# ultralytics/yolov5

Measured on NVIDIA H100. Metric: images/sec @640 (forward + NMS), higher is better.
Workload: dtype bf16

## Files before the change

include/y5b200.h:

```cpp
#ifndef Y5B200_H
#define Y5B200_H
#include <stdint.h>

#if defined(__GNUC__)
#define Y5_API __attribute__((visibility("default")))
#else
#define Y5_API
#endif

#ifdef __cplusplus
extern "C" {
#endif

#define Y5_F16 0
#define Y5_BF16 1
#define Y5_F32 2
#define Y5_U8 3

#define Y5_E_INVALID (-1)
#define Y5_E_UNSUPPORTED (-2)
#define Y5_E_DRIVER (-3)

#define Y5_ACT_NONE 0
#define Y5_ACT_SILU 1
// ... 3 lines not shown
int64_t y5_launch_count(void);

typedef struct y5_conv_desc {
    const void* in;
    int32_t in_pitch;
    int32_t batch, in_h, in_w, in_c;
    const void* weight;
    const float* bias;
    void* out;
    int32_t out_pitch;
    int32_t out_c;
    const void* residual;
    int32_t res_pitch;
    int32_t ksize, stride, pad;
    int32_t act;
    int32_t dtype;
    int32_t block_k;
    int32_t block_n;
    int32_t kw;
    int32_t pad_w;
    int64_t in_x_stride;
    int64_t in_y_stride;
    int64_t in_n_stride;
    int32_t a_mode;
    int32_t reserved;
} y5_conv_desc;

int y5_conv_pick(int32_t in_c, int32_t out_c, int64_t m_rows, int32_t* block_k, int32_t* block_n);

typedef struct y5_conv_plan y5_conv_plan;
int y5_conv_plan_create(const y5_conv_desc* desc, y5_conv_plan** plan);
int y5_conv_plan_run(const y5_conv_plan* plan, void* stream);
void y5_conv_plan_destroy(y5_conv_plan* plan);
int y5_conv_bn_silu_fwd(const y5_conv_desc* desc, void* stream);
int y5_conv_direct_fwd(const y5_conv_desc* desc, void* stream);

typedef struct y5_detect_desc {
    const void* in;
    int32_t in_pitch;
    int32_t batch, ny, nx, in_c;
    const void* weight;
    const float* bias;
    void* raw;
    void* z;
    int32_t z_rows, z_row0;
    int32_t na, no, nc;
    float stride;
    float anchor_wh[8];
    int32_t dtype;
    int32_t block_k;
} y5_detect_desc;
typedef struct y5_detect_plan y5_detect_plan;
int y5_detect_plan_create(const y5_detect_desc* desc, y5_detect_plan** plan);
int y5_detect_plan_run(const y5_detect_plan* plan, void* stream);
int y5_detect_plan_run_to(const y5_detect_plan* plan, void* raw, void* z, void* stream);
void y5_detect_plan_destroy(y5_detect_plan* plan);

int y5_stem_s2d(const void* img, int32_t img_dtype, void* out, int32_t out_dtype, int32_t batch, int32_t h, int32_t w,
                int32_t out_row_px, int32_t out_x_off, void* stream);
int y5_sppf_pool(const void* x, int32_t x_pitch, void* y1, void* y2, void* y3, int32_t y_pitch, int32_t batch, int32_t h,
                 int32_t w, int32_t c, int32_t ksize, int32_t dtype, void* stream);
int y5_upsample2x(const void* x, int32_t x_pitch, void* y, int32_t y_pitch, int32_t batch, int32_t h, int32_t w, int32_t c,
                  int32_t dtype, void* stream);
int y5_copy_view(const void* x, int32_t x_pitch, void* y, int32_t y_pitch, int64_t pixels, int32_t c, int32_t dtype,
                 void* stream);
int y5_nhwc_to_nchw(const void* x, int32_t x_pitch, void* y, int32_t batch, int32_t h, int32_t w, int32_t c, int32_t dtype,
// ... 277 lines not shown
```

yolov5_b200/_lib.py:

```python
from __future__ import annotations

import ctypes as C
import os

import torch

_HERE = os.path.dirname(os.path.abspath(__file__))
LIB_PATH = os.environ.get("Y5B200_LIB") or os.path.join(_HERE, "liby5b200.so")

Y5_F16, Y5_BF16, Y5_F32, Y5_U8 = 0, 1, 2, 3
ACT_NONE, ACT_SILU = 0, 1

_DTYPE = {torch.float16: Y5_F16, torch.bfloat16: Y5_BF16, torch.float32: Y5_F32, torch.uint8: Y5_U8}


def dtype_code(dt: torch.dtype) -> int:
    try:
        return _DTYPE[dt]
    except KeyError:
        raise TypeError(f"y5b200: unsupported dtype {dt}") from None


class ConvDesc(C.Structure):
    _fields_ = [
# ... 109 lines not shown
    ]


class AugLabel(C.Structure):
    _fields_ = [
        ("cls", C.c_float), ("x", C.c_float), ("y", C.c_float), ("w", C.c_float), ("h", C.c_float),
        ("tile_w", C.c_float), ("tile_h", C.c_float), ("pad_w", C.c_float), ("pad_h", C.c_float),
        ("image", C.c_int32), ("mosaic", C.c_int32), ("flags", C.c_int32),
    ]


AUG_CLIP, AUG_IN_XYXY, AUG_OUT_XYXY = 1, 2, 4


class AugSegment(C.Structure):
    _fields_ = [("point_offset", C.c_int32), ("n_points", C.c_int32)]


SEG_POINTS, SEG_I32 = 1000, 4

OPT_INV_SCALE, OPT_MAX_NORM, OPT_EMA_DECAY, OPT_EMA_TAU, OPT_EMA_UPDATES, OPT_OUT_NORM, OPT_OUT_SKIPPED, OPT_GROUPS = 0, 1, 2, 3, 4, 5, 6, 8
ADAM_LR, ADAM_BETA1, ADAM_BETA2, ADAM_EPS, ADAM_WEIGHT_DECAY, ADAM_DECOUPLED, ADAM_STRIDE = 0, 1, 2, 3, 4, 5, 8

_P = C.c_void_p
_I32, _I64, _F = C.c_int32, C.c_int64, C.c_float
SIGNATURES = {
    "y5_version": (_I32, []),
    "y5_last_error": (C.c_char_p, []),
    "y5_launch_count": (_I64, []),
    "y5_conv_pick": (_I32, [_I32, _I32, _I64, C.POINTER(_I32), C.POINTER(_I32)]),
    "y5_conv_plan_create": (_I32, [C.POINTER(ConvDesc), C.POINTER(_P)]),
    "y5_conv_plan_run": (_I32, [_P, _P]),
    "y5_conv_plan_destroy": (None, [_P]),
    "y5_conv_bn_silu_fwd": (_I32, [C.POINTER(ConvDesc), _P]),
    "y5_conv_direct_fwd": (_I32, [C.POINTER(ConvDesc), _P]),
    "y5_detect_plan_create": (_I32, [C.POINTER(DetectDesc), C.POINTER(_P)]),
    "y5_detect_plan_run": (_I32, [_P, _P]),
    "y5_detect_plan_run_to": (_I32, [_P, _P, _P, _P]),
    "y5_detect_plan_destroy": (None, [_P]),
    "y5_stem_s2d": (_I32, [_P, _I32, _P, _I32, _I32, _I32, _I32, _I32, _I32, _P]),
    "y5_sppf_pool": (_I32, [_P, _I32, _P, _P, _P, _I32, _I32, _I32, _I32, _I32, _I32, _I32, _P]),
    "y5_upsample2x": (_I32, [_P, _I32, _P, _I32, _I32, _I32, _I32, _I32, _I32, _P]),
    "y5_copy_view": (_I32, [_P, _I32, _P, _I32, _I64, _I32, _I32, _P]),
    "y5_nhwc_to_nchw": (_I32, [_P, _I32, _P, _I32, _I32, _I32, _I32, _I32, _P]),
    "y5_nms_workspace_bytes": (_I64, [C.POINTER(NmsParams)]),
    "y5_nms_batched": (_I32, [C.POINTER(NmsParams), _P, _P, _P, _P, _P, _I64, _P]),
    "y5_box_iou": (_I32, [_P, _I32, _P, _I32, _F, _P, _P]),
    "y5_loss_workspace_bytes": (_I64, [C.POINTER(LossParams)]),
    "y5_loss_fwd_bwd": (_I32, [C.POINTER(LossParams), C.POINTER(_P), _P, _P, _P, C.POINTER(_P), _P, _I64, _P]),
    "y5_loss_read_targets": (_I32, [C.POINTER(LossParams), _P, _I32, _P, _P, _P, _P]),
    "y5_seg_loss_workspace_bytes": (_I64, [C.POINTER(LossParams)]),
    "y5_seg_loss_fwd_bwd_scaled": (_I32, [C.POINTER(LossParams), C.POINTER(_P), _P, _P, _P, _I32, _I64, _I64, _I64, _I64, _I32, _I32, _I32,
                                          _P, _I32, _I32, _I32, _I32, _P, C.POINTER(_P), _P, _P, _P, _I64, _P]),
    "y5_seg_loss_read_targets": (_I32, [C.POINTER(LossParams), _P, _I32, _P, _P, _P, _P]),
    "y5_conv_wgrad": (_I32, [C.POINTER(WgradDesc), _P]),
    "y5_bn_workspace_bytes": (_I64, [_I32]),
    "y5_bn_stats": (_I32, [_P, _I32, _I64, _I32, _I32, _P, _P]),
    "y5_bn_act_fwd": (_I32, [_P, _I32, _P, _I32, _I64, _I32, _I32, _P, _P, _P, _P, _I32, _P, _F, _F, _P, _P, _P, _I32, _P]),
    "y5_upsample2x_bwd": (_I32, [_P, _I32, _P, _I32, _I32, _I32, _I32, _I32, _I32, _P]),
    "y5_sppf_bwd_workspace_bytes": (_I64, [_I32, _I32, _I32, _I32]),
    "y5_sppf_pool_bwd": (_I32, [_P, _I32, _P, _I32, _P, _I32, _I32, _I32, _I32, _I32, _I32, _I32, _P, _P]),
    "y5_bn_act_bwd": (_I32, [_P, _I32, _P, _I32, _P, _I32, _I64, _I32, _I32, _P, _P, _P, _P, _I32, _P, _P, _P, _P]),
    "y5_col_sum": (_I32, [_P, _I32, _I64, _I32, _I32, _P, _P, _P]),
    "y5_weight_pack": (_I32, [_P, _I32, _I32, _I32, _I32, _P, _I32, _P, _I32, _I32, _P]),
    "y5_weight_pack_chunk_elems": (_I32, []),
    "y5_weight_pack_multi": (_I32, [_P, _P, _P, _I32, _I32, _P]),
# ... 75 lines not shown
```

yolov5_b200/csrc/conv_gemm.cu:

```cuda
#include <cstdio>
#include <cstdlib>
#include <cstring>
#include <mutex>

#include "../../include/y5b200.h"
#include "common.cuh"
#include "host_util.h"
#include "wgmma.cuh"

namespace y5 {

constexpr int kBlockM = 128;
constexpr int kConsumers = 2;
constexpr int kConsumerThreads = 128 * kConsumers;
constexpr int kThreads = 128 + kConsumerThreads;
constexpr int kMaxStages = 8;
constexpr int kHeadN = 128;

enum AMode { A_LINEAR = 0, A_IM2COL = 1, A_PATCH = 2 };

struct ConvParams {
    int M, N;
    int num_m_tiles;
    int num_m_super, num_n_tiles;
    int kh, kw, c_chunks;
    int block_k;
    int a_mode;
    int Ho, Wo, HoWo, stride, pad_h, pad_w;
    int tw, th, tiles_x, tiles_y;
    int b_grouped;
    int patch_pw;
    int cluster_n;
    uint32_t stg_bytes;
    uint32_t b_sub_bytes;
    float rcp_per_img, rcp_tiles_x, rcp_HoWo, rcp_Wo;
    int a_stages, b_stages;
    uint32_t a_sub_bytes, a_stage_bytes, b_stage_bytes;
    int is_bf16, act;
    const float* bias;
    int bias_n;
    void* out;
    int out_pitch;
    const void* res;
    int res_pitch;
    void* raw;
    void* z;
    int na, no, nc, nx, z_rows, z_row0;
    float det_stride;
    float anchor_wh[8];
};

struct SmemLayout {
    uint32_t off_a, off_b, off_out, off_bias, off_bars, total;
};

__host__ __device__ inline SmemLayout smem_layout(int epi, int no, int bias_n, int a_stages, int b_stages, uint32_t a_bytes,
                                                   uint32_t b_bytes, uint32_t stg_bytes) {
    SmemLayout L;
    uint32_t o = 0;
    L.off_a = o;
    o += a_stages * a_bytes;
    L.off_b = o;
    o += b_stages * b_bytes;
    o = (o + 1023) & ~1023u;
    L.off_out = o;
    if (epi == 1) o += 4 * ((kBlockM * no * 2 + 1023) & ~1023u);
    else o += stg_bytes;
    L.off_bias = o;
    o += ((bias_n + 3) & ~3) * 4;
    o = (o + 7) & ~7u;
    L.off_bars = o;
    o += 4 * kMaxStages * 8;
    L.total = o;
    return L;
}

__device__ __forceinline__ int fdiv(int n, int d, float rd) {
    if (n >= (1 << 23)) return n / d;
    int q = __float2int_rz(__int2float_rz(n) * rd);
    const int r = n - q * d;
    if (r >= d) ++q;
    else if (r < 0) --q;
    return q;
}

template <int BLOCK_N, int MT, int KS, bool BF16>
__device__ __forceinline__ void mma_batch(float (&acc)[MT][BLOCK_N / 2], uint32_t a_lo, uint32_t a_sub16, uint32_t a_hi, uint32_t b_lo,
                                          uint32_t b_hi, uint32_t scale_first) {
    wgmma_fence();
#pragma unroll
    for (int k = 0; k < KS; ++k)
#pragma unroll
        for (int mi = 0; mi < MT; ++mi)
            Wgmma<BLOCK_N>::template run<BF16, 0, 0>(acc[mi], gmma_desc(a_lo + mi * a_sub16 + 2 * k, a_hi), gmma_desc(b_lo + 2 * k, b_hi),
                                                     k == 0 ? scale_first : 1u);
    wgmma_commit();
}

template <int BLOCK_N, int EPI, int MT, bool OPT, bool BF16>
__global__ void __launch_bounds__(kThreads, 1)
conv_gemm_kernel(const __grid_constant__ CUtensorMap tmA, const __grid_constant__ CUtensorMap tmB, const ConvParams p) {
    static_assert(MT * BLOCK_N <= 256, "accumulators: at most 128 fp32 registers per consumer thread");
    constexpr int kAcc = BLOCK_N / 2;

    extern __shared__ __align__(1024) uint8_t smem_raw[];
    uint8_t* smem = reinterpret_cast<uint8_t*>((reinterpret_cast<uintptr_t>(smem_raw) + 1023) & ~uintptr_t(1023));
    const SmemLayout L = smem_layout(EPI, p.no, p.bias_n, p.a_stages, p.b_stages, p.a_stage_bytes, p.b_stage_bytes, p.stg_bytes);
    uint8_t* sA = smem + L.off_a;
    uint8_t* sB = smem + L.off_b;
    float* sBias = reinterpret_cast<float*>(smem + L.off_bias);
    uint64_t* a_full = reinterpret_cast<uint64_t*>(smem + L.off_bars);
    uint64_t* a_empty = a_full + kMaxStages;
    uint64_t* b_full = a_empty + kMaxStages;
    uint64_t* b_empty = b_full + kMaxStages;

    const int warp = threadIdx.x >> 5;
    const int lane = threadIdx.x & 31;
    const int csize = OPT ? static_cast<int>(cluster_nctarank()) : 1;
    const uint32_t crank = OPT ? cluster_ctarank() : 0u;

    if (threadIdx.x == 0) {
        tma_prefetch_desc(&tmA);
        tma_prefetch_desc(&tmB);
        for (int s = 0; s < kMaxStages; ++s) {
            mbar_init(&a_full[s], 1);
            mbar_init(&a_empty[s], kConsumers);
            mbar_init(&b_full[s], 1);
            mbar_init(&b_empty[s], kConsumers * csize);
        }
        fence_barrier_init();
    }
    if (threadIdx.x >= 128)
        for (int i = threadIdx.x - 128; i < p.bias_n; i += kConsumerThreads) {
            const float b = i < p.N ? __ldg(p.bias + i) : 0.0f;
            sBias[i] = (EPI == 0 && p.act) ? 0.5f * b : b;
        }
    __syncthreads();
    if (csize > 1) cluster_sync_all();
    griddep_wait();
    griddep_launch_dependents();

    const int nn = p.num_n_tiles;
    const int num_tiles = ((p.num_m_super + csize - 1) / csize) * nn;
    const int tile0 = blockIdx.x / csize, tile_step = gridDim.x / csize;
    const uint32_t row_bytes = p.block_k * 2;
    const bool patch = p.a_mode == A_PATCH;
    const bool wide = OPT && p.patch_pw > 0;
    const int grp = wide ? p.kh * p.kw : (patch ? p.kh : 1);
    const int num_groups = wide ? p.c_chunks : (patch ? p.c_chunks * p.kw : p.kh * p.kw * p.c_chunks);

    if (warp < 4) {
        setmaxnreg_dec<56>();
    }
    if (warp == 0) {
        int as = 0, bs = 0;
        uint32_t aph = 0, bph = 0;
        for (int tile = tile0; tile < num_tiles; tile += tile_step) {
            const int ms = (tile / nn) * csize + static_cast<int>(crank);
            const int n0 = (tile - (tile / nn) * nn) * BLOCK_N;
            int img[MT], y0[MT], x0[MT];
#pragma unroll
            for (int mi = 0; mi < MT; ++mi) {
                const int mt = ms * MT + mi;
                img[mi] = y0[mi] = x0[mi] = 0;
                if (p.a_mode == A_IM2COL) {
                    const int m0 = mt * kBlockM;
                    img[mi] = fdiv(m0, p.HoWo, p.rcp_HoWo);
                    const int rem = m0 - img[mi] * p.HoWo;
                    const int oy = fdiv(rem, p.Wo, p.rcp_Wo);
                    y0[mi] = oy * p.stride - p.pad_h;
                    x0[mi] = (rem - oy * p.Wo) * p.stride - p.pad_w;
                } else if (patch) {
                    const int per_img = p.tiles_x * p.tiles_y;
                    img[mi] = fdiv(mt, per_img, p.rcp_per_img);
                    const int rem = mt - img[mi] * per_img;
                    const int ty = fdiv(rem, p.tiles_x, p.rcp_tiles_x);
                    y0[mi] = ty * p.th - p.pad_h;
                    x0[mi] = (rem - ty * p.tiles_x) * p.tw - p.pad_w;
                }
            }
            auto issue_group = [&](int cc, int s, int r0) {
                mbar_wait(&a_empty[as], aph ^ 1);
                if (elect_one()) {
                    mbar_arrive_expect_tx(&a_full[as], p.a_stage_bytes);
#pragma unroll
                    for (int mi = 0; mi < MT; ++mi) {
                        uint8_t* a_dst = sA + as * p.a_stage_bytes + mi * p.a_sub_bytes;
                        if (wide) {
                            if (mi == 0) tma_load_4d(&tmA, &a_full[as], a_dst, cc * p.block_k, x0[0], y0[0], img[0]);
                        } else if (p.a_mode == A_LINEAR) tma_load_2d(&tmA, &a_full[as], a_dst, cc * p.block_k, (ms * MT + mi) * kBlockM);
                        else if (p.a_mode == A_IM2COL)
                            tma_load_im2col_4d(&tmA, &a_full[as], a_dst, cc * p.block_k, x0[mi], y0[mi], img[mi], static_cast<uint16_t>(s),
                                               static_cast<uint16_t>(r0));
                        else tma_load_4d(&tmA, &a_full[as], a_dst, cc * p.block_k, x0[mi] + s, y0[mi], img[mi]);
                    }
                }
                __syncwarp();
                if (++as == p.a_stages) { as = 0; aph ^= 1; }
                for (int j = 0; j < grp; ++j) {
                    const int r = patch ? j : r0;
                    const int kb = wide ? j * p.c_chunks + cc : (r * p.kw + s) * p.c_chunks + cc;
                    const bool stage_first = !p.b_grouped || j == 0, stage_last = !p.b_grouped || j == grp - 1;
                    if (stage_first) mbar_wait(&b_empty[bs], bph ^ 1);
                    if (elect_one()) {
                        if (stage_first) mbar_arrive_expect_tx(&b_full[bs], p.b_stage_bytes);
                        uint8_t* b_dst = sB + bs * p.b_stage_bytes + (p.b_grouped ? j * p.b_sub_bytes : 0u);
                        if (csize == 1) tma_load_2d(&tmB, &b_full[bs], b_dst, kb * p.block_k, n0);
                        else {
                            const int slice_rows = BLOCK_N / csize;
                            tma_load_2d_mcast(&tmB, &b_full[bs], b_dst + crank * slice_rows * row_bytes, kb * p.block_k,
                                              n0 + static_cast<int>(crank) * slice_rows, static_cast<uint16_t>((1u << csize) - 1u));
                        }
                    }
                    __syncwarp();
                    if (stage_last && ++bs == p.b_stages) { bs = 0; bph ^= 1; }
                }
            };
            if (wide) {
                for (int cc = 0; cc < p.c_chunks; ++cc) issue_group(cc, 0, 0);
            } else if (patch) {
                for (int cc = 0; cc < p.c_chunks; ++cc)
                    for (int s = 0; s < p.kw; ++s) issue_group(cc, s, 0);
            } else {
                for (int r = 0; r < p.kh; ++r)
                    for (int s = 0; s < p.kw; ++s)
                        for (int cc = 0; cc < p.c_chunks; ++cc) issue_group(cc, s, r);
            }
        }
    } else if (warp >= 4) {
    setmaxnreg_inc<224>();
    const int wg = (warp >> 2) - 1;
    const int ct = threadIdx.x - 128;
    const int wrow = wg * 64 + (warp & 3) * 16 + (lane >> 2);
    const int ccol = 2 * (lane & 3);
    const bool signal = (threadIdx.x & 127) == 0;
    constexpr bool bf16 = BF16;
    const uint32_t dhi = gmma_desc_hi(row_bytes);
    const uint32_t a_hi = wide ? (dhi & ~0x3FFFu) | (((static_cast<uint32_t>(p.patch_pw) * row_bytes) >> 4) & 0x3FFFu) : dhi;
    const uint32_t a_base = gmma_desc_lo(smem_u32(sA) + (wide ? wg * 8 * p.patch_pw : wg * 64) * row_bytes), b_base = gmma_desc_lo(smem_u32(sB));
    const uint32_t row16 = row_bytes >> 4;
    const uint32_t a_stage16 = p.a_stage_bytes >> 4, b_stage16 = p.b_stage_bytes >> 4, a_sub16 = p.a_sub_bytes >> 4;
    const uint32_t b_sub16 = p.b_sub_bytes >> 4;
    const uint32_t a_shift16 = patch ? (p.tw * row_bytes) >> 4 : 0;
    const int k_steps = p.block_k / 16;
    const int per_img = p.tiles_x * p.tiles_y;
    const int tw_shift = patch ? __ffs(p.tw) - 1 : 0;
    int as = 0, bs = 0, head_set = 0;
    uint32_t aph = 0, bph = 0;
    float acc[MT][kAcc];
#pragma unroll
    for (int mi = 0; mi < MT; ++mi)
#pragma unroll
        for (int i = 0; i < kAcc; ++i) acc[mi][i] = 0.0f;

    int pend_as = 0, pend_bs = 0;
    bool pend_a_last = false, pend_b_last = false;
    auto release_pending = [&]() {
        if (!signal) return;
        if (pend_b_last) {
            if (csize == 1) mbar_arrive(&b_empty[pend_bs]);
            else
                for (int r = 0; r < csize; ++r) mbar_arrive_cluster(mapa_u32(&b_empty[pend_bs], static_cast<uint32_t>(r)));
        }
        if (pend_a_last) mbar_arrive(&a_empty[pend_as]);
    };

    for (int tile = tile0; tile < num_tiles; tile += tile_step) {
        const int ms = (tile / nn) * csize + static_cast<int>(crank);
        const int nt = tile - (tile / nn) * nn;
        const int n0 = nt * BLOCK_N;
        for (int g = 0; g < num_groups; ++g) {
            mbar_wait(&a_full[as], aph);
            const uint32_t a_stage_lo = a_base + as * a_stage16;
            uint32_t a_lo = a_stage_lo;
            for (int j = 0; j < grp; ++j) {
                if (wide) {
                    const int tr = j / p.kw, ts = j - tr * p.kw;
                    a_lo = a_stage_lo + (tr * p.patch_pw + ts) * row16;
                }
                const bool stage_first = !p.b_grouped || j == 0, stage_last = !p.b_grouped || j == grp - 1;
                if (stage_first) mbar_wait(&b_full[bs], bph);
                const uint32_t b_lo = b_base + bs * b_stage16 + (p.b_grouped ? j * b_sub16 : 0u);
                const uint32_t scale_first = (g | j) != 0 ? 1u : 0u;
#pragma unroll
                for (int mi = 0; mi < MT; ++mi) fence_regs(acc[mi]);
                switch (k_steps) {
                    case 4: mma_batch<BLOCK_N, MT, 4, BF16>(acc, a_lo, a_sub16, a_hi, b_lo, dhi, scale_first); break;
                    case 2: mma_batch<BLOCK_N, MT, 2, BF16>(acc, a_lo, a_sub16, a_hi, b_lo, dhi, scale_first); break;
                    default: mma_batch<BLOCK_N, MT, 1, BF16>(acc, a_lo, a_sub16, a_hi, b_lo, dhi, scale_first); break;
                }
                wgmma_wait<1>();
#pragma unroll
                for (int mi = 0; mi < MT; ++mi) fence_regs(acc[mi]);
                if (g | j) release_pending();
                pend_as = as;
                pend_a_last = j == grp - 1;
                pend_bs = bs;
                pend_b_last = stage_last;
                if (stage_last && ++bs == p.b_stages) { bs = 0; bph ^= 1; }
                a_lo += a_shift16;
            }
            if (++as == p.a_stages) { as = 0; aph ^= 1; }
        }
        wgmma_wait<0>();
#pragma unroll
        for (int mi = 0; mi < MT; ++mi) fence_regs(acc[mi]);
        release_pending();

        if (EPI == 0) {
            const bool staged = OPT && p.stg_bytes != 0;
            const uint32_t stg_pitch = BLOCK_N * 2 + 16;
            uint8_t* stg = smem + L.off_out + wg * 64 * stg_pitch;
            auto pixel_of = [&](int mt, int row) -> long long {
                if (patch) {
                    const int img = fdiv(mt, per_img, p.rcp_per_img);
                    const int rem = mt - img * per_img;
                    const int tyi = fdiv(rem, p.tiles_x, p.rcp_tiles_x);
                    const int oy = tyi * p.th + (row >> tw_shift), ox = (rem - tyi * p.tiles_x) * p.tw + (row & ((1 << tw_shift) - 1));
                    return (mt < p.num_m_tiles && oy < p.Ho && ox < p.Wo) ? static_cast<long long>(img) * p.HoWo + oy * p.Wo + ox : -1;
                }
                const long long m = static_cast<long long>(mt) * kBlockM + row;
                return m < p.M ? m : -1;
            };
            constexpr int kRows = 2 * MT, kWords = (OPT ? 128 : 256) / BLOCK_N;
            constexpr int kBatch = kWords < 1 ? 1 : (kWords < kRows ? kWords : kRows);
            const bool has_res = p.res != nullptr;
#pragma unroll
            for (int q0 = 0; q0 < kRows; q0 += kBatch) {
                uint32_t rv[kBatch][BLOCK_N / 8];
                long long gp[kBatch];
#pragma unroll
                for (int q = 0; q < kBatch; ++q) gp[q] = pixel_of(ms * MT + (q0 + q) / 2, wrow + 8 * ((q0 + q) & 1));
                if (has_res) {
#pragma unroll
                    for (int q = 0; q < kBatch; ++q) {
                        const uint16_t* rp = reinterpret_cast<const uint16_t*>(p.res) + (gp[q] < 0 ? 0 : gp[q] * p.res_pitch) + n0 + ccol;
#pragma unroll
                        for (int j = 0; j < BLOCK_N / 8; ++j)
                            rv[q][j] = (gp[q] >= 0 && n0 + 8 * j < p.N) ? *reinterpret_cast<const uint32_t*>(rp + 8 * j) : 0u;
                    }
// ... 166 lines not shown

int pick_block_n(int out_c, int64_t m_rows) {
    int bn, mt;
    pick_tile(out_c, m_rows > 0 ? (m_rows + kBlockM - 1) / kBlockM : 1, &bn, &mt);
    return bn;
}

template <int BN, int EPI, int MT, bool OPT>
cudaError_t launch_conv(const CUtensorMap& a, const CUtensorMap& b, const ConvParams& p, int grid, int cluster, uint32_t smem,
                        cudaStream_t st) {
    auto* kernel = p.is_bf16 ? conv_gemm_kernel<BN, EPI, MT, OPT, true> : conv_gemm_kernel<BN, EPI, MT, OPT, false>;
    const cudaError_t attr_err = ensure_dyn_smem(reinterpret_cast<const void*>(kernel), 227 * 1024);
    if (attr_err != cudaSuccess) return attr_err;
    count_launch();
    if (cluster == 1) return launch_pdl(kernel, dim3(grid), dim3(kThreads), smem, st, a, b, p);
    static const bool pdl = [] { const char* e = getenv("Y5_PDL"); return !(e && e[0] == '0'); }();
    cudaLaunchConfig_t cfg{};
    cfg.gridDim = dim3(grid);
    cfg.blockDim = dim3(kThreads);
    cfg.dynamicSmemBytes = smem;
    cfg.stream = st;
    cudaLaunchAttribute attr[2];
    attr[0].id = cudaLaunchAttributeClusterDimension;
    attr[0].val.clusterDim.x = cluster;
    attr[0].val.clusterDim.y = 1;
    attr[0].val.clusterDim.z = 1;
    attr[1].id = cudaLaunchAttributeProgrammaticStreamSerialization;
    attr[1].val.programmaticStreamSerializationAllowed = 1;
    cfg.attrs = attr;
    cfg.numAttrs = pdl ? 2 : 1;
    return cudaLaunchKernelEx(&cfg, kernel, a, b, p);
}

struct PlanCommon {
    CUtensorMap tmA, tmB;
    ConvParams p;
    int block_n, epi, mt, grid, cluster;
    uint32_t smem_bytes;
};

int finish_plan(PlanCommon& pc, int block_n, int epi, int mt, int cluster = 1) {
    ConvParams& p = pc.p;
    p.cluster_n = cluster;
    p.a_stage_bytes = mt * p.a_sub_bytes;
    if (p.patch_pw > 0) p.a_stage_bytes = static_cast<uint32_t>(p.th + p.kh - 1) * p.patch_pw * p.block_k * 2;
    p.num_m_super = (p.num_m_tiles + mt - 1) / mt;
    p.num_n_tiles = epi == 1 ? p.na : (p.N + block_n - 1) / block_n;
    p.bias_n = p.num_n_tiles * block_n;
    const uint32_t budget = 225 * 1024 - 1024;
    const bool patch = p.a_mode == A_PATCH;
    int a_st = 0, b_st = 0;
    if (!patch) {
        for (int s = kMaxStages; s >= 2; --s)
            if (smem_layout(epi, p.no, p.bias_n, s, s, p.a_stage_bytes, p.b_stage_bytes, p.stg_bytes).total <= budget) { a_st = b_st = s; break; }
    } else {
        const int b_min = p.b_grouped ? 2 : 3, b_max = p.b_grouped ? 4 : kMaxStages;
        for (int a = 3; a >= 2 && !a_st; --a)
            for (int b = b_max; b >= b_min; --b)
                if (smem_layout(epi, p.no, p.bias_n, a, b, p.a_stage_bytes, p.b_stage_bytes, p.stg_bytes).total <= budget) { a_st = a; b_st = b; break; }
    }
    if (a_st < 2 || b_st < 2) return set_error(Y5_E_UNSUPPORTED, "conv tile does not fit shared memory (block_n %d a %u b %u)", block_n,
                                                p.a_stage_bytes, p.b_stage_bytes);
    p.a_stages = a_st;
    p.b_stages = b_st;
    pc.smem_bytes = smem_layout(epi, p.no, p.bias_n, a_st, b_st, p.a_stage_bytes, p.b_stage_bytes, p.stg_bytes).total + 1024;
    pc.block_n = block_n;
    pc.epi = epi;
    pc.mt = mt;
    pc.cluster = cluster;
    const long long tiles = static_cast<long long>((p.num_m_super + cluster - 1) / cluster) * p.num_n_tiles;
    const int max_clusters = sm_count() / cluster;
    pc.grid = static_cast<int>(tiles < max_clusters ? tiles : max_clusters) * cluster;
    return 0;
}

int run_plan(const PlanCommon& pc, cudaStream_t st) {
    cudaError_t e = cudaErrorInvalidValue;
    const bool opt = pc.cluster > 1 || pc.p.patch_pw > 0 || pc.p.stg_bytes > 0;
    const int key = (opt ? 100000 : 0) + pc.epi * 10000 + pc.block_n * 10 + pc.mt;
    switch (key) {
        case 324: e = launch_conv<32, 0, 4, false>(pc.tmA, pc.tmB, pc.p, pc.grid, pc.cluster, pc.smem_bytes, st); break;
        case 642: e = launch_conv<64, 0, 2, false>(pc.tmA, pc.tmB, pc.p, pc.grid, pc.cluster, pc.smem_bytes, st); break;
        case 1281: e = launch_conv<128, 0, 1, false>(pc.tmA, pc.tmB, pc.p, pc.grid, pc.cluster, pc.smem_bytes, st); break;
        case 1282: e = launch_conv<128, 0, 2, false>(pc.tmA, pc.tmB, pc.p, pc.grid, pc.cluster, pc.smem_bytes, st); break;
        case 2561: e = launch_conv<256, 0, 1, false>(pc.tmA, pc.tmB, pc.p, pc.grid, pc.cluster, pc.smem_bytes, st); break;
        case 11281: e = launch_conv<kHeadN, 1, 1, false>(pc.tmA, pc.tmB, pc.p, pc.grid, pc.cluster, pc.smem_bytes, st); break;
        case 100324: e = launch_conv<32, 0, 4, true>(pc.tmA, pc.tmB, pc.p, pc.grid, pc.cluster, pc.smem_bytes, st); break;
        case 100642: e = launch_conv<64, 0, 2, true>(pc.tmA, pc.tmB, pc.p, pc.grid, pc.cluster, pc.smem_bytes, st); break;
        case 101281: e = launch_conv<128, 0, 1, true>(pc.tmA, pc.tmB, pc.p, pc.grid, pc.cluster, pc.smem_bytes, st); break;
        case 101282: e = launch_conv<128, 0, 2, true>(pc.tmA, pc.tmB, pc.p, pc.grid, pc.cluster, pc.smem_bytes, st); break;
        case 102561: e = launch_conv<256, 0, 1, true>(pc.tmA, pc.tmB, pc.p, pc.grid, pc.cluster, pc.smem_bytes, st); break;
        default: return set_error(Y5_E_UNSUPPORTED, "conv: no kernel for block_n %d mt %d epi %d", pc.block_n, pc.mt, pc.epi);
    }
    if (e != cudaSuccess) return set_error(int(e), "conv_gemm launch failed: %s", cudaGetErrorString(e));
    return 0;
}

bool aligned16(const void* p) { return (reinterpret_cast<uintptr_t>(p) & 15) == 0; }

struct Geo {
    int kh, kw, pad_h, pad_w, Ho, Wo;
    long long xs, ys, ns;
};
Geo geometry(const y5_conv_desc* d) {
    Geo g;
    g.kh = d->ksize;
    g.kw = d->kw ? d->kw : d->ksize;
    g.pad_h = d->pad;
    g.pad_w = d->kw ? d->pad_w : d->pad;
    g.xs = d->in_x_stride ? d->in_x_stride : d->in_pitch;
    g.ys = d->in_y_stride ? d->in_y_stride : static_cast<long long>(d->in_w) * g.xs;
    g.ns = d->in_n_stride ? d->in_n_stride : static_cast<long long>(d->in_h) * g.ys;
    g.Ho = (d->in_h + 2 * g.pad_h - g.kh) / d->stride + 1;
    g.Wo = (d->in_w + 2 * g.pad_w - g.kw) / d->stride + 1;
    return g;
}

}

struct y5_conv_plan {
    PlanCommon pc;
};
struct y5_detect_plan {
    PlanCommon pc;
};

extern "C" Y5_API int y5_conv_pick(int32_t in_c, int32_t out_c, int64_t m_rows, int32_t* block_k, int32_t* block_n) {
    if (in_c <= 0 || out_c <= 0) return set_error(Y5_E_INVALID, "y5_conv_pick: non-positive channel count");
    if (block_k) *block_k = pick_block_k(in_c);
    if (block_n) *block_n = pick_block_n(out_c, m_rows);
    return 0;
// ... 106 lines not shown
            const double eff8 = (double)g.Wo * g.Ho / ((double)tx8 * 8 * ty16 * 16);
            if ((d->reserved & 128) && !(d->reserved & 32) && row_bytes == 128 && g.kw > 1 && (mt_sel == 1 || (mt_sel == 2 && tx8 % 2 == 0)) &&
                eff8 >= best_eff - 1e-9) {
                p.tw = 8;
                p.th = 16;
                p.patch_pw = 8 * mt_sel + 8;
            }
        }
        if (!p.patch_pw && g.kh > 1 && bn <= 128) {
            p.b_grouped = 1;
            p.b_stage_bytes = g.kh * p.b_sub_bytes;
        }
        p.tiles_x = (g.Wo + p.tw - 1) / p.tw;
        p.tiles_y = (g.Ho + p.th - 1) / p.th;
        p.rcp_tiles_x = 1.0f / static_cast<float>(p.tiles_x);
        p.rcp_per_img = 1.0f / static_cast<float>(p.tiles_x * p.tiles_y);
        p.num_m_tiles = d->batch * p.tiles_x * p.tiles_y;
        p.a_sub_bytes = p.patch_pw ? 8 * row_bytes : (p.th + g.kh - 1) * p.tw * row_bytes;
        cuuint64_t dims[4] = {(cuuint64_t)d->in_c, (cuuint64_t)d->in_w, (cuuint64_t)d->in_h, (cuuint64_t)d->batch};
        cuuint64_t str[3] = {(cuuint64_t)g.xs * 2, (cuuint64_t)g.ys * 2, (cuuint64_t)g.ns * 2};
        cuuint32_t box[4] = {(cuuint32_t)bk, (cuuint32_t)(p.patch_pw ? p.patch_pw : p.tw), (cuuint32_t)(p.th + g.kh - 1), 1};
        e = encode_tiled(&pc.tmA, d->dtype, d->in, 4, dims, str, box, sw, "A patch");
    }
    if (e) { delete plan; return e; }
    const uint64_t ktot = static_cast<uint64_t>(p.kh) * p.kw * p.c_chunks * bk;
    {
        cuuint64_t dims[2] = {ktot, (cuuint64_t)d->out_c};
        cuuint64_t str[1] = {ktot * 2};
        cuuint32_t box[2] = {(cuuint32_t)bk, (cuuint32_t)(bn / cl_sel)};
        e = encode_tiled(&pc.tmB, d->dtype, d->weight, 2, dims, str, box, sw, "B");
    }
    if (e) { delete plan; return e; }
    p.stg_bytes = ((d->reserved & 8) && !(d->reserved & 16)) ? static_cast<uint32_t>(kConsumers * 64 * (bn * 2 + 16)) : 0u;
    int e2 = finish_plan(pc, bn, 0, mt_sel, cl_sel);
    if (e2 && p.stg_bytes) {
        p.stg_bytes = 0;
        e2 = finish_plan(pc, bn, 0, mt_sel, cl_sel);
    }
    if (e2) { delete plan; return e2; }
    *out = plan;
    return 0;
}

extern "C" Y5_API int y5_conv_plan_run(const y5_conv_plan* plan, void* stream) {
    if (!plan) return set_error(Y5_E_INVALID, "conv: null plan");
    return run_plan(plan->pc, static_cast<cudaStream_t>(stream));
}
extern "C" Y5_API void y5_conv_plan_destroy(y5_conv_plan* plan) { delete plan; }

extern "C" Y5_API int y5_conv_bn_silu_fwd(const y5_conv_desc* d, void* stream) {
    y5_conv_plan* plan = nullptr;
    if (int e = y5_conv_plan_create(d, &plan)) return e;
    const int e = y5_conv_plan_run(plan, stream);
    y5_conv_plan_destroy(plan);
    return e;
}

extern "C" Y5_API int y5_conv_direct_fwd(const y5_conv_desc* d, void* stream) {
    if (int e = validate_conv(d)) return e;
    const Geo g = geometry(d);
    const int bk = d->block_k ? d->block_k : pick_block_k(d->in_c);
    const int cin_pad = (d->in_c + bk - 1) / bk * bk;
    const long long total = static_cast<long long>(d->batch) * g.Ho * g.Wo * d->out_c;
    const int threads = 256;
    const long long blocks = (total + threads - 1) / threads;
    conv_direct_kernel<<<static_cast<unsigned>(blocks), threads, 0, static_cast<cudaStream_t>(stream)>>>(
        static_cast<const uint16_t*>(d->in), g.xs, g.ys, g.ns, d->batch, d->in_h, d->in_w, d->in_c, static_cast<const uint16_t*>(d->weight),
        cin_pad, d->bias, static_cast<uint16_t*>(d->out), d->out_pitch, d->out_c, static_cast<const uint16_t*>(d->residual), d->res_pitch,
        g.kh, g.kw, d->stride, g.pad_h, g.pad_w, g.Ho, g.Wo, d->act, d->dtype == Y5_BF16);
    count_launch();
    cudaError_t e = cudaGetLastError();
    if (e != cudaSuccess) return set_error(int(e), "conv_direct launch failed: %s", cudaGetErrorString(e));
    return 0;
}

extern "C" Y5_API int y5_detect_plan_create(const y5_detect_desc* d, y5_detect_plan** out) {
    if (!out) return set_error(Y5_E_INVALID, "detect: null plan out");
    *out = nullptr;
    if (!d || !d->in || !d->weight || !d->bias || !d->raw || !d->z) return set_error(Y5_E_INVALID, "detect: null pointer");
    if (d->dtype != Y5_F16 && d->dtype != Y5_BF16) return set_error(Y5_E_UNSUPPORTED, "detect: dtype must be fp16/bf16");
    if (d->na < 1 || d->na > 4 || d->no < 6 || d->no > kHeadN || d->nc < 1 || 5 + d->nc > d->no)
// ... 61 lines not shown
```

yolov5_b200/engine.py:

```python
from __future__ import annotations

import ctypes as C
import math
import os

import torch

from . import _lib
from ._lib import ConvDesc, DetectDesc

BN_EPS_DEFAULT = 1e-3


class View:

    __slots__ = ("buf", "coff", "c", "h", "w")

    def __init__(self, buf: torch.Tensor, coff: int, c: int):
        self.buf, self.coff, self.c = buf, coff, c
        self.h, self.w = buf.shape[1], buf.shape[2]

    @property
    def pitch(self) -> int:
        return self.buf.shape[3]
# ... 44 lines not shown
    return out


class _Op:

    __slots__ = ("fn", "args", "name", "keep")

    def __init__(self, name, fn, args, keep=()):
        self.name, self.fn, self.args, self.keep = name, fn, args, keep

    def run(self, stream: int):
        _lib.check(self.fn(*self.args, C.c_void_p(stream)), self.name)


class Program:

    def __init__(self, module, batch: int, height: int, width: int, dtype: torch.dtype, device, in_channels=None):
        if dtype not in (torch.float16, torch.bfloat16):
            raise TypeError(f"y5b200 engine computes in fp16 or bf16, got {dtype} (call model.half() / .bfloat16())")
        self.lib = _lib.lib()
        self.module = module
        self.B, self.H, self.W = batch, height, width
        self.dtype, self.device = dtype, torch.device(device)
        self.dt_code = _lib.dtype_code(dtype)
        self.ops: list[_Op] = []
        self.head_ops: list = []
        self._plans: list = []
        self._keep: list = []
        self.graph = None
        self.flops = 0
        self.act_bytes = 0
        self.weight_bytes = 0
        self.in_channels = in_channels
        self._build()

    def new_buf(self, h: int, w: int, c: int) -> torch.Tensor:
        t = torch.zeros(self.B, h, w, _pad8(c), dtype=self.dtype, device=self.device)
        self._keep.append(t)
        return t

    def new_view(self, h: int, w: int, c: int) -> View:
        return View(self.new_buf(h, w, c), 0, c)

    def block_k(self, cin: int, cout: int, m_rows: int) -> int:
        bk = C.c_int32()
        _lib.check(self.lib.y5_conv_pick(cin, cout, m_rows, C.byref(bk), None), "conv_pick")
        return bk.value

    def fold_pack(self, parts, m_rows: int):
        cin, kh, kw = parts[0][0].shape[1:]
        cout = sum(w.shape[0] for w, _, _ in parts)
        bk = self.block_k(cin, cout, m_rows)
        ipad = (cin + bk - 1) // bk * bk
        wp = torch.empty(cout, kh, kw, ipad, dtype=self.dtype, device=self.device)
        bias = torch.empty(cout, dtype=torch.float32, device=self.device)
        self.fold_pack_into(parts, wp, bias, 0, ipad)
        return wp, bias, bk

    def fold_pack_into(self, parts, wp, bias, row0: int, ipad: int, pad_rows_to: int | None = None):
        st = C.c_void_p(_lib.stream_ptr(self.device))
        es = wp.element_size()
        for w, cb, bn in parts:
            w = w.detach()
            if not w.is_contiguous():
                w = w.contiguous()
            if w.device != self.device:
                raise RuntimeError("y5b200: module parameters and the input must live on the same CUDA device")
# ... 32 lines not shown
        m_rows = self.B * ho * wo
        bk, bn = C.c_int32(), C.c_int32()
        bn.value = int(os.environ.get("Y5_FORCE_BLOCK_N", "0"))
        if packed is None:
            assert w_fp32.shape == (cout, cin, k, kw), (w_fp32.shape, cout, cin, k, kw)
            bk.value = self.block_k(cin, cout, m_rows)
            wp = pack_weight(w_fp32, bk.value, self.dtype)
            bias = b_fp32.to(torch.float32).contiguous()
        else:
            wp, bias, bk.value, pc = packed
            assert pc == cin and wp.shape[0] == cout and wp.shape[1:3] == (k, kw), (name, wp.shape, cout, cin, k, kw)
        self._keep += [wp, bias]
        d = ConvDesc()
        if virt is None:
            d.inp, d.in_pitch = x.ptr, x.pitch
        else:
            d.inp, d.in_pitch = virt["ptr"], virt["x_stride"]
            d.in_x_stride, d.in_y_stride, d.in_n_stride = virt["x_stride"], virt["y_stride"], virt["n_stride"]
            d.kw, d.pad_w = kw, virt["pad_w"]
        d.batch, d.in_h, d.in_w, d.in_c = self.B, in_h, in_w, cin
        d.weight, d.bias = wp.data_ptr(), bias.data_ptr()
        d.out, d.out_pitch, d.out_c = out.ptr, out.pitch, cout
        d.residual = residual.ptr if residual is not None else None
        d.res_pitch = residual.pitch if residual is not None else 0
        d.ksize, d.stride, d.pad = k, s, p
        d.act = _lib.ACT_SILU if act else _lib.ACT_NONE
        d.dtype, d.block_k, d.block_n = self.dt_code, bk.value, bn.value
        d.a_mode = int(os.environ.get("Y5_FORCE_A_MODE", "0"))
        if d.a_mode == 2 and s != 1:
            d.a_mode = 0
        plan = C.c_void_p()
        _lib.check(self.lib.y5_conv_plan_create(C.byref(d), C.byref(plan)), f"conv_plan_create[{name}]")
        self._plans.append((self.lib.y5_conv_plan_destroy, plan))
        self.ops.append(_Op(name, self.lib.y5_conv_plan_run, (plan,)))
        if virt is None:
            self.flops += 2 * m_rows * cout * cin * k * k
            self.act_bytes += 2 * (self.B * x.h * x.w * x.c + m_rows * cout)
            self.weight_bytes += 2 * cout * cin * k * k

    def conv_module(self, m, x: View, out: View, residual: View | None = None, name="conv"):
        k, s, p = m.conv.kernel_size[0], m.conv.stride[0], m.conv.padding[0]
        act = isinstance(m.act, torch.nn.SiLU)
        if not act and not isinstance(m.act, torch.nn.Identity):
            raise NotImplementedError(f"y5b200: activation {type(m.act).__name__} (only SiLU / Identity are built)")
        if m.conv.groups != 1 or m.conv.dilation[0] != 1:
            raise NotImplementedError("y5b200: grouped / dilated convolutions are outside the YOLOv5 n..x hot path")
        ho, wo = (x.h + 2 * p - k) // s + 1, (x.w + 2 * p - k) // s + 1
        wp, bias, bk = self.fold_pack([(m.conv.weight, m.conv.bias, getattr(m, "bn", None))], self.B * ho * wo)
        self.conv(x, out, None, None, k, s, p, act, residual, name, packed=(wp, bias, bk, x.c))

    def out_hw(self, m, x: View):
        k, s, p = m.conv.kernel_size[0], m.conv.stride[0], m.conv.padding[0]
        return (x.h + 2 * p - k) // s + 1, (x.w + 2 * p - k) // s + 1

    def lower_conv(self, m, x, out: View | None, name):
        from .models.common import Conv

        k, s, p, cin = m.conv.kernel_size[0], m.conv.stride[0], m.conv.padding[0], m.conv.in_channels
        if isinstance(x, torch.Tensor):
            if not (k == 6 and s == 2 and p == 2 and cin == 3):
                raise NotImplementedError("y5b200: the first layer must be the YOLOv5 v6 stem Conv(3, c, 6, 2, 2)")
            if self.H % 2 or self.W % 2:
                raise ValueError("y5b200: image height and width must be even")
            h2, w2 = self.H // 2, self.W // 2
            s2d_buf = torch.zeros(self.B, h2, w2 + 2, 16, dtype=self.dtype, device=self.device)
            self._keep.append(s2d_buf)
# ... 329 lines not shown
```

Baseline: 3070.

## Add stream-K split of tail conv tiles with workspace fixup

```diff
diff --git a/include/y5b200.h b/include/y5b200.h
--- a/include/y5b200.h
+++ b/include/y5b200.h
@@ -59,6 +59,8 @@
 int y5_conv_plan_create(const y5_conv_desc* desc, y5_conv_plan** plan);
 int y5_conv_plan_run(const y5_conv_plan* plan, void* stream);
 void y5_conv_plan_destroy(y5_conv_plan* plan);
+int64_t y5_conv_plan_workspace_bytes(const y5_conv_plan* plan);
+int y5_conv_plan_set_workspace(y5_conv_plan* plan, void* workspace, int64_t workspace_bytes);
 int y5_conv_bn_silu_fwd(const y5_conv_desc* desc, void* stream);
 int y5_conv_direct_fwd(const y5_conv_desc* desc, void* stream);
 
diff --git a/yolov5_b200/_lib.py b/yolov5_b200/_lib.py
--- a/yolov5_b200/_lib.py
+++ b/yolov5_b200/_lib.py
@@ -165,6 +165,8 @@
     "y5_conv_plan_create": (_I32, [C.POINTER(ConvDesc), C.POINTER(_P)]),
     "y5_conv_plan_run": (_I32, [_P, _P]),
     "y5_conv_plan_destroy": (None, [_P]),
+    "y5_conv_plan_workspace_bytes": (_I64, [_P]),
+    "y5_conv_plan_set_workspace": (_I32, [_P, _P, _I64]),
     "y5_conv_bn_silu_fwd": (_I32, [C.POINTER(ConvDesc), _P]),
     "y5_conv_direct_fwd": (_I32, [C.POINTER(ConvDesc), _P]),
     "y5_detect_plan_create": (_I32, [C.POINTER(DetectDesc), C.POINTER(_P)]),
diff --git a/yolov5_b200/csrc/conv_gemm.cu b/yolov5_b200/csrc/conv_gemm.cu
--- a/yolov5_b200/csrc/conv_gemm.cu
+++ b/yolov5_b200/csrc/conv_gemm.cu
@@ -36,6 +36,10 @@
     float rcp_per_img, rcp_tiles_x, rcp_HoWo, rcp_Wo;
     int a_stages, b_stages;
     uint32_t a_sub_bytes, a_stage_bytes, b_stage_bytes;
+    int sk_tiles, sk_base, sk_rem;
+    int num_tiles, units;
+    float rcp_units;
+    float* sk_ws;
     int is_bf16, act;
     const float* bias;
     int bias_n;
@@ -84,6 +88,18 @@
     return q;
 }
 
+__device__ __forceinline__ int ld_acquire_gpu(const int* p) {
+    int v;
+    asm volatile("ld.acquire.gpu.global.b32 %0, [%1];" : "=r"(v) : "l"(p) : "memory");
+    return v;
+}
+__device__ __forceinline__ void st_release_gpu(int* p, int v) { asm volatile("st.release.gpu.global.b32 [%0], %1;" ::"l"(p), "r"(v) : "memory"); }
+__device__ __forceinline__ int cta_id() {
+    int v;
+    asm volatile("mov.u32 %0, %%ctaid.x;" : "=r"(v));
+    return v;
+}
+
 template <int BLOCK_N, int MT, int KS, bool BF16>
 __device__ __forceinline__ void mma_batch(float (&acc)[MT][BLOCK_N / 2], uint32_t a_lo, uint32_t a_sub16, uint32_t a_hi, uint32_t b_lo,
                                           uint32_t b_hi, uint32_t scale_first) {
@@ -141,13 +157,30 @@
     griddep_launch_dependents();
 
     const int nn = p.num_n_tiles;
-    const int num_tiles = ((p.num_m_super + csize - 1) / csize) * nn;
-    const int tile0 = blockIdx.x / csize, tile_step = gridDim.x / csize;
+    const int tile_step = gridDim.x >> (csize >> 1);
     const uint32_t row_bytes = p.block_k * 2;
     const bool patch = p.a_mode == A_PATCH;
     const bool wide = OPT && p.patch_pw > 0;
     const int grp = wide ? p.kh * p.kw : (patch ? p.kh : 1);
-    const int num_groups = wide ? p.c_chunks : (patch ? p.c_chunks * p.kw : p.kh * p.kw * p.c_chunks);
+    const int num_groups = p.units;
+
+    auto seg_start = [&](int c) { return c * p.sk_base + min(c, p.sk_rem); };
+    auto next_item = [&](int& cur, int& tile, int& g0, int& g1) -> bool {
+        const int sk_begin = seg_start(cta_id());
+        if (cur > sk_begin) {
+            tile = fdiv(cur - 1, num_groups, p.rcp_units);
+            const int t0 = tile * num_groups;
+            g0 = max(t0, sk_begin) - t0;
+            g1 = cur - t0;
+            cur = t0 + g0;
+            return true;
+        }
+        tile = p.sk_tiles + cta_id() / csize + (sk_begin - cur) * tile_step;
+        g0 = 0;
+        g1 = num_groups;
+        --cur;
+        return tile < p.num_tiles;
+    };
 
     if (warp < 4) {
         setmaxnreg_dec<56>();
@@ -155,7 +188,7 @@
     if (warp == 0) {
         int as = 0, bs = 0;
         uint32_t aph = 0, bph = 0;
-        for (int tile = tile0; tile < num_tiles; tile += tile_step) {
+        for (int cur = seg_start(cta_id() + 1), tile, g0, g1; next_item(cur, tile, g0, g1);) {
             const int ms = (tile / nn) * csize + static_cast<int>(crank);
             const int n0 = (tile - (tile / nn) * nn) * BLOCK_N;
             int img[MT], y0[MT], x0[MT];
@@ -216,15 +249,17 @@
                     if (stage_last && ++bs == p.b_stages) { bs = 0; bph ^= 1; }
                 }
             };
-            if (wide) {
-                for (int cc = 0; cc < p.c_chunks; ++cc) issue_group(cc, 0, 0);
-            } else if (patch) {
-                for (int cc = 0; cc < p.c_chunks; ++cc)
-                    for (int s = 0; s < p.kw; ++s) issue_group(cc, s, 0);
-            } else {
-                for (int r = 0; r < p.kh; ++r)
-                    for (int s = 0; s < p.kw; ++s)
-                        for (int cc = 0; cc < p.c_chunks; ++cc) issue_group(cc, s, r);
+            int cc = 0, s = 0, r = 0;
+            if (g0 > 0) {
+                if (wide) cc = g0;
+                else if (patch) { cc = g0 / p.kw; s = g0 - cc * p.kw; }
+                else { const int rs = g0 / p.c_chunks; cc = g0 - rs * p.c_chunks; r = rs / p.kw; s = rs - r * p.kw; }
+            }
+            for (int g = g0; g < g1; ++g) {
+                issue_group(cc, s, r);
+                if (wide) ++cc;
+                else if (patch) { if (++s == p.kw) { s = 0; ++cc; } }
+                else if (++cc == p.c_chunks) { cc = 0; if (++s == p.kw) { s = 0; ++r; } }
             }
         }
     } else if (warp >= 4) {
@@ -265,11 +300,32 @@
         if (pend_a_last) mbar_arrive(&a_empty[pend_as]);
     };
 
-    for (int tile = tile0; tile < num_tiles; tile += tile_step) {
+    for (int cur = seg_start(cta_id() + 1), tile, g0, g1; next_item(cur, tile, g0, g1);) {
         const int ms = (tile / nn) * csize + static_cast<int>(crank);
         const int nt = tile - (tile / nn) * nn;
         const int n0 = nt * BLOCK_N;
-        for (int g = 0; g < num_groups; ++g) {
+        constexpr int kVec = MT * kAcc / 4;
+        float4* slots = reinterpret_cast<float4*>(p.sk_ws);
+        int* flags = reinterpret_cast<int*>(p.sk_ws + static_cast<size_t>(gridDim.x) * kBlockM * MT * BLOCK_N);
+        if (EPI == 0 && g0 > 0) {
+            const int prev = cta_id() - 1;
+            if (ct == 0) {
+                while (ld_acquire_gpu(flags + prev) == 0) __nanosleep(32);
+                flags[prev] = 0;
+            }
+            named_bar_sync(1, kConsumerThreads);
+            const float4* slot = slots + (prev * kVec * kConsumerThreads + ct);
+#pragma unroll
+            for (int v = 0; v < kVec; ++v) {
+                const int mi = (4 * v) / kAcc, i = (4 * v) % kAcc;
+                const float4 t = __ldcg(slot + v * kConsumerThreads);
+                acc[mi][i] = t.x;
+                acc[mi][i + 1] = t.y;
+                acc[mi][i + 2] = t.z;
+                acc[mi][i + 3] = t.w;
+            }
+        }
+        for (int g = g0; g < g1; ++g) {
             mbar_wait(&a_full[as], aph);
             const uint32_t a_stage_lo = a_base + as * a_stage16;
             uint32_t a_lo = a_stage_lo;
@@ -281,7 +337,8 @@
                 const bool stage_first = !p.b_grouped || j == 0, stage_last = !p.b_grouped || j == grp - 1;
                 if (stage_first) mbar_wait(&b_full[bs], bph);
                 const uint32_t b_lo = b_base + bs * b_stage16 + (p.b_grouped ? j * b_sub16 : 0u);
-                const uint32_t scale_first = (g | j) != 0 ? 1u : 0u;
+                const bool first = g == g0 && j == 0;
+                const uint32_t scale_first = first && g0 == 0 ? 0u : 1u;
 #pragma unroll
                 for (int mi = 0; mi < MT; ++mi) fence_regs(acc[mi]);
                 switch (k_steps) {
@@ -292,7 +349,7 @@
                 wgmma_wait<1>();
 #pragma unroll
                 for (int mi = 0; mi < MT; ++mi) fence_regs(acc[mi]);
-                if (g | j) release_pending();
+                if (!first) release_pending();
                 pend_as = as;
                 pend_a_last = j == grp - 1;
                 pend_bs = bs;
@@ -306,6 +363,19 @@
 #pragma unroll
         for (int mi = 0; mi < MT; ++mi) fence_regs(acc[mi]);
         release_pending();
+
+        if (EPI == 0 && g1 < num_groups) {
+            float4* slot = slots + (cta_id() * kVec * kConsumerThreads + ct);
+#pragma unroll
+            for (int v = 0; v < kVec; ++v) {
+                const int mi = (4 * v) / kAcc, i = (4 * v) % kAcc;
+                __stcg(slot + v * kConsumerThreads, make_float4(acc[mi][i], acc[mi][i + 1], acc[mi][i + 2], acc[mi][i + 3]));
+            }
+            __threadfence();
+            named_bar_sync(1, kConsumerThreads);
+            if (ct == 0) st_release_gpu(flags + cta_id(), 1);
+            continue;
+        }
 
         if (EPI == 0) {
             const bool staged = OPT && p.stg_bytes != 0;
@@ -538,14 +608,20 @@
     return cudaLaunchKernelEx(&cfg, kernel, a, b, p);
 }
 
+bool aligned16(const void* p) { return (reinterpret_cast<uintptr_t>(p) & 15) == 0; }
+
 struct PlanCommon {
     CUtensorMap tmA, tmB;
     ConvParams p;
     int block_n, epi, mt, grid, cluster;
     uint32_t smem_bytes;
+    int dp_grid, sk_tiles, sk_units;
+    int64_t ws_bytes;
 };
 
-int finish_plan(PlanCommon& pc, int block_n, int epi, int mt, int cluster = 1) {
+constexpr int kFixupK = 768;
+
+int finish_plan(PlanCommon& pc, int block_n, int epi, int mt, int cluster = 1, bool allow_sk = false) {
     ConvParams& p = pc.p;
     p.cluster_n = cluster;
     p.a_stage_bytes = mt * p.a_sub_bytes;
@@ -576,7 +652,45 @@
     pc.cluster = cluster;
     const long long tiles = static_cast<long long>((p.num_m_super + cluster - 1) / cluster) * p.num_n_tiles;
     const int max_clusters = sm_count() / cluster;
-    pc.grid = static_cast<int>(tiles < max_clusters ? tiles : max_clusters) * cluster;
+    pc.grid = pc.dp_grid = static_cast<int>(tiles < max_clusters ? tiles : max_clusters) * cluster;
+    pc.sk_tiles = pc.sk_units = 0;
+    pc.ws_bytes = 0;
+    const int sms = sm_count();
+    const int units = p.patch_pw > 0 ? p.c_chunks : (patch ? p.c_chunks * p.kw : p.kh * p.kw * p.c_chunks);
+    p.num_tiles = static_cast<int>(tiles);
+    p.units = units;
+    const long long tile_k = static_cast<long long>(p.kh) * p.kw * p.c_chunks * p.block_k;
+    const long long tail = tiles % sms;
+    if (allow_sk && epi == 0 && cluster == 1 && tiles > sms && tail != 0 &&
+        (sms - tail) * tile_k > static_cast<long long>(sms) * kFixupK) {
+        const long long sk_tiles = tail + sms;
+        if (sk_tiles * units < (1LL << 23)) {
+            pc.sk_tiles = static_cast<int>(sk_tiles);
+            pc.sk_units = static_cast<int>(sk_tiles * units);
+            const int64_t slot = static_cast<int64_t>(kBlockM) * mt * block_n * 4;
+            pc.ws_bytes = sms * slot + ((sms * 4 + 255) & ~255);
+        }
+    }
+    p.rcp_units = 1.0f / static_cast<float>(units);
+    return 0;
+}
+
+int set_workspace(PlanCommon& pc, void* ws, int64_t bytes) {
+    ConvParams& p = pc.p;
+    if (ws && pc.ws_bytes > 0) {
+        if (bytes < pc.ws_bytes) return set_error(Y5_E_INVALID, "conv: workspace of %lld bytes, the plan needs %lld", (long long)bytes,
+                                                  (long long)pc.ws_bytes);
+        if (!aligned16(ws)) return set_error(Y5_E_INVALID, "conv: workspace must be 16-byte aligned");
+        pc.grid = sm_count();
+        p.sk_ws = static_cast<float*>(ws);
+        p.sk_tiles = pc.sk_tiles;
+        p.sk_base = pc.sk_units / pc.grid;
+        p.sk_rem = pc.sk_units % pc.grid;
+    } else {
+        pc.grid = pc.dp_grid;
+        p.sk_ws = nullptr;
+        p.sk_tiles = p.sk_base = p.sk_rem = 0;
+    }
     return 0;
 }
 
@@ -601,8 +715,6 @@
     if (e != cudaSuccess) return set_error(int(e), "conv_gemm launch failed: %s", cudaGetErrorString(e));
     return 0;
 }
-
-bool aligned16(const void* p) { return (reinterpret_cast<uintptr_t>(p) & 15) == 0; }
 
 struct Geo {
     int kh, kw, pad_h, pad_w, Ho, Wo;
@@ -775,10 +887,11 @@
     }
     if (e) { delete plan; return e; }
     p.stg_bytes = ((d->reserved & 8) && !(d->reserved & 16)) ? static_cast<uint32_t>(kConsumers * 64 * (bn * 2 + 16)) : 0u;
-    int e2 = finish_plan(pc, bn, 0, mt_sel, cl_sel);
+    const bool allow_sk = !(d->reserved & 64);
+    int e2 = finish_plan(pc, bn, 0, mt_sel, cl_sel, allow_sk);
     if (e2 && p.stg_bytes) {
         p.stg_bytes = 0;
-        e2 = finish_plan(pc, bn, 0, mt_sel, cl_sel);
+        e2 = finish_plan(pc, bn, 0, mt_sel, cl_sel, allow_sk);
     }
     if (e2) { delete plan; return e2; }
     *out = plan;
@@ -790,6 +903,14 @@
     return run_plan(plan->pc, static_cast<cudaStream_t>(stream));
 }
 extern "C" Y5_API void y5_conv_plan_destroy(y5_conv_plan* plan) { delete plan; }
+extern "C" Y5_API int64_t y5_conv_plan_workspace_bytes(const y5_conv_plan* plan) {
+    if (!plan) return set_error(Y5_E_INVALID, "conv: null plan");
+    return plan->pc.ws_bytes;
+}
+extern "C" Y5_API int y5_conv_plan_set_workspace(y5_conv_plan* plan, void* ws, int64_t bytes) {
+    if (!plan) return set_error(Y5_E_INVALID, "conv: null plan");
+    return set_workspace(plan->pc, ws, bytes);
+}
 
 extern "C" Y5_API int y5_conv_bn_silu_fwd(const y5_conv_desc* d, void* stream) {
     y5_conv_plan* plan = nullptr;
diff --git a/yolov5_b200/engine.py b/yolov5_b200/engine.py
--- a/yolov5_b200/engine.py
+++ b/yolov5_b200/engine.py
@@ -100,7 +100,14 @@
         self.act_bytes = 0
         self.weight_bytes = 0
         self.in_channels = in_channels
+        self._conv_plans: list = []
         self._build()
+        ws_bytes = max((int(self.lib.y5_conv_plan_workspace_bytes(h)) for h in self._conv_plans), default=0)
+        if ws_bytes > 0:
+            ws = torch.zeros(ws_bytes, dtype=torch.uint8, device=self.device)
+            self._keep.append(ws)
+            for h in self._conv_plans:
+                _lib.check(self.lib.y5_conv_plan_set_workspace(h, ws.data_ptr(), ws_bytes), "conv_plan_set_workspace")
 
     def new_buf(self, h: int, w: int, c: int) -> torch.Tensor:
         t = torch.zeros(self.B, h, w, _pad8(c), dtype=self.dtype, device=self.device)
@@ -199,6 +206,7 @@
         plan = C.c_void_p()
         _lib.check(self.lib.y5_conv_plan_create(C.byref(d), C.byref(plan)), f"conv_plan_create[{name}]")
         self._plans.append((self.lib.y5_conv_plan_destroy, plan))
+        self._conv_plans.append(plan)
         self.ops.append(_Op(name, self.lib.y5_conv_plan_run, (plan,)))
         if virt is None:
             self.flops += 2 * m_rows * cout * cin * k * k
```

Result: slower. 2785, median of 6 (-9.3%).
